# santurini/vsrlab

Hardware: AMD Instinct MI355X
Metric: LR frames/sec fwd+bwd, BasicVSR 4x 540p 7-frame clip, 1->8 MI355X (higher is better)
Workload: dtype bf16; 1 GPU; BasicVSR(mid=64,res_blocks=30,x4) fwd+Charbonnier+bwd+clip+Adam, 540x960->2160x3840, 7-frame clip, 2 clips per GPU (BASELINE configs[1]); clips_per_gpu=2, frames=7, res_blocks=30, parallelism=single GPU, arena=full, train_flow=False, trunk_chains=True

## Files before the change

### vsrlab_amd/csrc/conv3x3_c64_tile.h

```cpp
#pragma once
#include "common.h"

constexpr int PTW = 32, PTH = 8, PNT = 512;
constexpr int PTWH = PTW + 2, PTHH = PTH + 2, PNPIX = PTHH * PTWH;
constexpr int W_BYTES = 9 * 64 * 64 * 2;
constexpr int IN_BYTES = PNPIX * 128;
constexpr int BIAS_OFF = W_BYTES + 2 * IN_BYTES;
constexpr int IN_CHUNKS = PNPIX * 8;
constexpr int NPIECE_T = (IN_CHUNKS + 63) / 64;
constexpr int NPIECE_W = (NPIECE_T + 3) / 4;
constexpr int WCH = 9 * 64 * 8 / 256;

typedef __attribute__((ext_vector_type(2))) __bf16 bf16x2_t;
typedef __attribute__((ext_vector_type(4))) unsigned u32x4_t;
typedef __attribute__((ext_vector_type(2))) unsigned u32x2_t;
#define GP(T, x) ((__attribute__((address_space(1))) T*)(x))

static __device__ __forceinline__ unsigned pk_bf16(float a, float b) {
    bf16x2_t p = {(bf16_t)a, (bf16_t)b};
    return __builtin_bit_cast(unsigned, p);
}
static __device__ __forceinline__ unsigned pk_max_i16(unsigned a, unsigned b) { unsigned r; asm("v_pk_max_i16 %0, %1, %2" : "=v"(r) : "v"(a), "v"(b)); return r; }
static __device__ __forceinline__ unsigned pk_min_u16(unsigned a, unsigned b) { unsigned r; asm("v_pk_min_u16 %0, %1, %2" : "=v"(r) : "v"(a), "v"(b)); return r; }
static __device__ __forceinline__ unsigned pk_mul_lo_u16(unsigned a, unsigned b) { unsigned r; asm("v_pk_mul_lo_u16 %0, %1, %2" : "=v"(r) : "v"(a), "v"(b)); return r; }
// ... 12 lines not shown
        *reinterpret_cast<u32x4_t*>((lds_w) + tap * 8192 + C64_W_SWIZZLED_BYTE(r, c)) = wv[i];                           \
    }

#define C64_DMA_REL(rel, w4, lane, in_step, src_oy, src_ox, WSs)                                                         \
    _Pragma("unroll") for (int i = 0; i < NPIECE_W; ++i) {                                                               \
        const int idx = ((w4) + 4 * i) * 64 + (lane);             \
        const int ty = idx / (8 * PTWH), rem = idx - ty * (8 * PTWH);                                                    \
        const int c = rem / PTWH, tx = rem - c * PTWH;                                                                   \
        const int dx = (tx - 1) * (in_step) + (src_ox);                                                                  \
        rel[i] = (((((ty - 1) * (in_step) + (src_oy)) * (WSs) + (dx >> 5)) * 8 + c) * 256 + (dx & 31) * 8) * 2;          \
    }
#define C64_GLDS16(src, dst, AUX)                                                                     \
    __builtin_amdgcn_global_load_lds((const __attribute__((address_space(1))) void*)(src),            \
                                     (__attribute__((address_space(3))) void*)(dst), 16, 0, AUX)
#define C64_DMA_TILE(AUX, rel, org, zsrc, dstb, w4, lane, ty0, tx0, H, W)                                                \
    if (ty0 >= 1 && ty0 + PTH < (H) && tx0 >= 1 && tx0 + PTW < (W)) {                   \
        _Pragma("unroll") for (int i = 0; i < NPIECE_W; ++i) {                                                           \
            const int piece = (w4) + 4 * i;                                                                              \
            if (piece < NPIECE_T && piece * 64 + (lane) < IN_CHUNKS) C64_GLDS16((org) + rel[i], (dstb) + piece * 1024, AUX); \
        }                                                                                                                \
    } else {                                                                     \
        _Pragma("unroll") for (int i = 0; i < NPIECE_W; ++i) {                                                           \
            const int piece = (w4) + 4 * i;                                                                              \
            const int idx = piece * 64 + (lane);                                                                         \
            const int ty = idx / (8 * PTWH), rem = idx - ty * (8 * PTWH);                                                \
            const int tx = rem % PTWH;                                                                                   \
            const int vy = ty0 + ty - 1, vx = tx0 + tx - 1;                                                              \
            const auto* s = (vy >= 0 && vy < (H) && vx >= 0 && vx < (W)) ? (org) + rel[i] : (zsrc);                      \
            if (piece < NPIECE_T && idx < IN_CHUNKS) C64_GLDS16(s, (dstb) + piece * 1024, AUX);                          \
        }                                                                                                                \
    }

#define C64_MFMA_LANE(w4, l15, q, pxl)                                                                                   \
    unsigned a_lo[2], a_hi[2];                                                                                           \
    _Pragma("unroll") for (int kk = 0; kk < 2; ++kk) {                                                                   \
        a_lo[kk] = (unsigned)C64_W_SWIZZLED_BYTE(l15, 4 * kk + (q));                                                     \
        a_hi[kk] = a_lo[kk] + 6 * 8192;                                                                                  \
    }                                                                                                                    \
    const int b_lane = (w4) * 2 * (PTWH * 128) + (q) * (PTWH * 16) + (pxl) * 16;
static __device__ __forceinline__ f32x4_t c64_bias_rows(const char* smem, int q, int mb) {
    return *reinterpret_cast<const f32x4_t*>(smem + BIAS_OFF + (mb * 16 + 4 * q) * 4);
}
#define C64_RES_IDENTITY(idA, l15, q)                                                                                    \
    bf16x8_t idA[2];                                                                                                     \
    _Pragma("unroll") for (int hb = 0; hb < 2; ++hb)                                                                     \
        _Pragma("unroll") for (int j = 0; j < 8; ++j) idA[hb][j] = (bf16_t)(((q) == ((l15) >> 2) && j == 4 * hb + ((l15) & 3)) ? 1.f : 0.f);
#define C64_ADD_RESIDUAL(acc, idA, rr)                                                                                 \
    _Pragma("unroll") for (int nb = 0; nb < 4; ++nb)                                                                   \
        _Pragma("unroll") for (int mb = 0; mb < 4; ++mb)                                                               \
            acc[mb][nb] = __builtin_amdgcn_mfma_f32_16x16x32_bf16(idA[mb & 1], __builtin_bit_cast(bf16x8_t, rr[mb >> 1][nb]), acc[mb][nb], 0, 0, 0);

#define C64_DSR(dst, addr, imm) asm volatile("ds_read_b128 %0, %1 offset:%2" : "=v"(dst) : "v"(addr), "i"(imm))
#define C64_LOADA(tap_, kk_, slot, mb)                                                                                 \
    C64_DSR(fa_[slot][mb], (tap_ < 6 ? a_lo[kk_] : a_hi[kk_]), (tap_ < 6 ? tap_ : tap_ - 6) * 8192 + (mb) * 2048);
#define C64_LOADB(ky_, kx_, kk_, slot, nb)                                                                             \
    C64_DSR(fb_[slot][nb], bb_, (((nb) >> 1) + ky_) * (PTWH * 128) + kk_ * (4 * PTWH * 16) + (((nb) & 1) * 16 + kx_) * 16);
#define C64_LOAD(s, slot)                                                                                              \
    {                                                                                                                  \
        constexpr int tap_ = (s) / 2, kk_ = (s) % 2, ky_ = tap_ / 3, kx_ = tap_ % 3;                                   \
        C64_LOADA(tap_, kk_, slot, 0) C64_LOADA(tap_, kk_, slot, 1) C64_LOADA(tap_, kk_, slot, 2) C64_LOADA(tap_, kk_, slot, 3) \
        C64_LOADB(ky_, kx_, kk_, slot, 0) C64_LOADB(ky_, kx_, kk_, slot, 1) C64_LOADB(ky_, kx_, kk_, slot, 2) C64_LOADB(ky_, kx_, kk_, slot, 3) \
    }
#define C64_MFMA(acc, bvec, s, mb, nb) acc[mb][nb] = __builtin_amdgcn_mfma_f32_16x16x32_bf16(fa_[(s) % 2][mb], fb_[(s) % 2][nb], (s) == 0 ? bvec[mb] : acc[mb][nb], 0, 0, 0);
#define C64_ML_A(acc, bvec, s, mb, nb, lmb)                                                                            \
    C64_MFMA(acc, bvec, s, mb, nb)                                                                                     \
    __builtin_amdgcn_sched_barrier(0);                       \
    if ((s) + 1 < 18) { constexpr int t1_ = ((s) + 1) / 2, k1_ = ((s) + 1) % 2; C64_LOADA(t1_, k1_, ((s) + 1) % 2, lmb) } \
    __builtin_amdgcn_sched_barrier(0);
#define C64_ML_B(acc, bvec, s, mb, nb, lnb)                                                                            \
    C64_MFMA(acc, bvec, s, mb, nb)                                                                                     \
    __builtin_amdgcn_sched_barrier(0);                                                                                 \
    if ((s) + 1 < 18) { constexpr int t1_ = ((s) + 1) / 2, k1_ = ((s) + 1) % 2; C64_LOADB(t1_ / 3, t1_ % 3, k1_, ((s) + 1) % 2, lnb) } \
    __builtin_amdgcn_sched_barrier(0);
#define C64_STEP(acc, bvec, s)                                                                                         \
    {                                                                                                                  \
        asm volatile("s_waitcnt lgkmcnt(0)" ::: "memory");                                 \
        __builtin_amdgcn_sched_barrier(0);                                                                             \
        C64_ML_A(acc, bvec, s, 0, 0, 0) C64_ML_A(acc, bvec, s, 0, 1, 1) C64_ML_A(acc, bvec, s, 0, 2, 2) C64_ML_A(acc, bvec, s, 0, 3, 3) \
        C64_ML_B(acc, bvec, s, 1, 0, 0) C64_ML_B(acc, bvec, s, 1, 1, 1) C64_ML_B(acc, bvec, s, 1, 2, 2) C64_ML_B(acc, bvec, s, 1, 3, 3) \
        C64_MFMA(acc, bvec, s, 2, 0) C64_MFMA(acc, bvec, s, 2, 1) C64_MFMA(acc, bvec, s, 2, 2) C64_MFMA(acc, bvec, s, 2, 3)  \
        C64_MFMA(acc, bvec, s, 3, 0) C64_MFMA(acc, bvec, s, 3, 1) C64_MFMA(acc, bvec, s, 3, 2) C64_MFMA(acc, bvec, s, 3, 3)  \
        __builtin_amdgcn_sched_barrier(0);                                                                             \
    }
#define C64_K_LOOP(acc, bvec, cur)                                                                                                    \
    {                                                                                                                  \
        bf16x8_t fa_[2][4], fb_[2][4];                                                                                 \
        const unsigned bb_ = (unsigned)(W_BYTES + (cur) * IN_BYTES + (b_lane));      \
        asm volatile("s_waitcnt lgkmcnt(0)" ::: "memory");                         \
        __builtin_amdgcn_sched_barrier(0);                                                                             \
        C64_LOAD(0, 0)                                                                                                 \
        C64_STEP(acc, bvec, 0) C64_STEP(acc, bvec, 1) C64_STEP(acc, bvec, 2) C64_STEP(acc, bvec, 3) C64_STEP(acc, bvec, 4) C64_STEP(acc, bvec, 5) \
        C64_STEP(acc, bvec, 6) C64_STEP(acc, bvec, 7) C64_STEP(acc, bvec, 8) C64_STEP(acc, bvec, 9) C64_STEP(acc, bvec, 10) C64_STEP(acc, bvec, 11) \
        C64_STEP(acc, bvec, 12) C64_STEP(acc, bvec, 13) C64_STEP(acc, bvec, 14) C64_STEP(acc, bvec, 15) C64_STEP(acc, bvec, 16) C64_STEP(acc, bvec, 17) \
    }

constexpr unsigned C64_K11 = 0x00010001u;
#define C64_ARM_PLAIN(ow, v)                                                                                             \
    _Pragma("unroll") for (int jj = 0; jj < 4; ++jj) ow[jj] = pk_bf16(v[2 * jj], v[2 * jj + 1]);
#define C64_ARM_RELU(ow, v, nb, sign_k)                                                                                  \
    _Pragma("unroll") for (int jj = 0; jj < 4; ++jj) {                                                                   \
        ow[jj] = pk_max_i16(pk_bf16(v[2 * jj], v[2 * jj + 1]), 0u);                                                      \
        sign_k |= pk_min_u16(ow[jj], C64_K11) << (4 * (nb) + jj);                                                        \
    }
#define C64_ARM_MASKED(ow, v, nb, wbits)                                                                                 \
    _Pragma("unroll") for (int jj = 0; jj < 4; ++jj)                                                                     \
        ow[jj] = pk_mul_lo_u16(pk_bf16(v[2 * jj], v[2 * jj + 1]), ((wbits) >> (4 * (nb) + jj)) & C64_K11);
static __device__ __forceinline__ long long c64_sign_word(int tile, int w4, int lane) { return (long long)tile * 256 + w4 * 64 + lane; }
```

### vsrlab_amd/csrc/conv3x3_chain.hip

```cpp
#include "conv3x3_c64_tile.h"
#include "kernels.h"
#include <atomic>
#include <type_traits>

namespace {

constexpr int CTL_OFF = BIAS_OFF + 256;
constexpr int P_LDS = CTL_OFF + 128;
constexpr int DMA_SC1 = 16;

#ifdef VSR_CLOCK
__device__ unsigned long long g_clk_chain[256 * 2];
#endif
#ifdef VSR_TEST_CHAIN_NO_PUBLISH
#define CHAIN_PUBLISH 0
#else
#define CHAIN_PUBLISH 1
#endif
__device__ uint4 g_chain_zero_chunk[2];
__device__ unsigned g_chain_timeouts;

typedef __attribute__((address_space(1))) unsigned gu32;
#define RLX_AGENT __ATOMIC_RELAXED, __HIP_MEMORY_SCOPE_AGENT

// ... 150 lines not shown
                if (__builtin_amdgcn_readfirstlane(s1[5]) == 0) {
                    (void)halo_wait(flg0 + 4 * ((long long)(l1 - 1) * tiles + (long long)n1 * per), ty1, tx1, nty, ntx, lane, err);
                    if (leader && lane == 0) s1[5] = 1;
                }
                __builtin_amdgcn_fence(__ATOMIC_ACQUIRE, "wavefront");
                issue(l1, n1, ty1, tx1, (k + 1) & 1);
            }
            if (leader) {
                int* s2 = ctl + 8 * ((k + 2) % 3);
                int it2 = -1, l2 = 0, n2 = 0, ty2 = 0, tx2 = 0;
                bool ok2 = false;
                if (fetch) {
                    asm volatile("s_waitcnt vmcnt(11)" : "+v"(nx) :: "memory");
                    static_assert(NPIECE_W == 11, "the counted wait above");
                    if (__builtin_amdgcn_readfirstlane((int)nx) == -1) asm volatile("s_waitcnt vmcnt(0)" : "+v"(nx) :: "memory");
                    it2 = chain_item((unsigned)__builtin_amdgcn_readfirstlane((int)nx), own, R, tiles, ntx, ka.nlayers);
                    if (it2 >= 0) {
                        l2 = it2 / tiles; const int r = it2 - l2 * tiles; n2 = r / per; const int r2 = r - n2 * per; ty2 = r2 / ntx; tx2 = r2 - ty2 * ntx;
                        ok2 = l2 == 0 || halo_ready(flg0 + 4 * ((long long)(l2 - 1) * tiles + (long long)n2 * per), ty2, tx2, nty, ntx, lane);
                    }
                }
                if (lane == 0) { s2[0] = it2; s2[1] = l2; s2[2] = n2; s2[3] = ty2; s2[4] = tx2; s2[5] = ok2 ? 1 : 0; }
            }
            asm volatile("s_waitcnt vmcnt(0)" ::: "memory");
            __syncthreads();
        }
    } else {
        u32x4_t wv[WCH];
        {
            const auto* wg = GP(const u32x4_t, base + (unsigned long long)ka.layer[ctl[1]].w * 256ull);
            C64_W_LOAD(wv, wg, tid & 255)
        }
        C64_MFMA_LANE(w4, l15, q, pxl)
        unsigned loff[4];
#pragma unroll
        for (int nb = 0; nb < 4; ++nb) {
            const int dx = (nb & 1) * 16 + pxl;
            loff[nb] = (((((w4 * 2 + (nb >> 1))) * WS + (dx >> 5)) * 8 + q) * 256 + (dx & 31) * 8) * 2;
        }
        C64_W_STORE(wv, lds_w, tid & 255)
        if (tid < 64) {
            const unsigned bo = ka.layer[ctl[1]].bias;
            reinterpret_cast<float*>(smem + BIAS_OFF)[tid] = bo != 0xffffffffu ? GP(const float, base + (unsigned long long)bo * 256ull)[pm_acc_chan(tid >> 4, tid & 15)] : 0.f;
        }
        asm volatile("s_waitcnt vmcnt(0)" ::: "memory");
        __syncthreads();
        f32x4_t bvec[4];
#pragma unroll
        for (int mb = 0; mb < 4; ++mb) bvec[mb] = c64_bias_rows(smem, q, mb);
        C64_RES_IDENTITY(idA, l15, q)

        int cur_layer = __builtin_amdgcn_readfirstlane(ctl[1]);
        unsigned long long p_dst, p_res, p_sbits, p_sout;
        int variant;
        auto layer_ptrs = [&](int l) {
            const ChainLayer L = ka.layer[l];
            p_dst = (unsigned long long)base + (unsigned long long)L.dst * 256ull;
            p_res = (unsigned long long)base + (unsigned long long)L.res * 256ull;
            p_sbits = (unsigned long long)base + (unsigned long long)L.sbits * 256ull;
            p_sout = L.sout != 0xffffffffu ? (unsigned long long)base + (unsigned long long)L.sout * 256ull : 0ull;
            variant = L.variant;
        };
        layer_ptrs(cur_layer);

        bool pending = false;
        gu32* pend_cnt = nullptr;
        int cur = 0;
        int item = __builtin_amdgcn_readfirstlane(ctl[0]), layer = cur_layer, tn = __builtin_amdgcn_readfirstlane(ctl[2]);
        int tyi = __builtin_amdgcn_readfirstlane(ctl[3]), txi = __builtin_amdgcn_readfirstlane(ctl[4]);
        for (int k = 0; item >= 0; ++k) {
            const int* sn = ctl + 8 * ((k + 1) % 3);
            int nx_item = -1, nx_layer = 0, nx_n = 0, nx_ty = 0, nx_tx = 0, nx_ok = 0;
            if (layer != cur_layer) {
                cur_layer = layer;
                layer_ptrs(layer);
                __syncthreads();
#pragma unroll
                for (int mb = 0; mb < 4; ++mb) bvec[mb] = c64_bias_rows(smem, q, mb);
            }
            const int tile = item - layer * tiles;
            const int ty0 = tyi * PTH, tx0 = txi * PTW;
            const long long tbase = (long long)tn * img + pm_off(ty0, tx0, 0, W, 64);
            const bool full = ty0 + PTH <= H && tx0 + PTW <= W;
            bool ok[4];
#pragma unroll
            for (int nb = 0; nb < 4; ++nb) ok[nb] = (tx0 + (nb & 1) * 16 + pxl < W) && (ty0 + w4 * 2 + (nb >> 1) < H);
            gu32* const my_cnt = flg0 + 4 * (long long)item + w4;

            auto body = [&](auto VC) {
                constexpr int V = decltype(VC)::value;
                constexpr bool HAS_RES = V == CHAIN_SKIP, BITS = V == CHAIN_MASK;
                u32x4_t rr[2][4];
                u32x2_t sbits = {0u, 0u};
                if (BITS) sbits = GP(const u32x2_t, p_sbits)[c64_sign_word(tile, w4, lane)];
                if (HAS_RES) {
                    const unsigned long long rbase = p_res + (unsigned long long)tbase * 2ull;
#pragma unroll
                    for (int nb = 0; nb < 4; ++nb) {
                        const unsigned lo = loff[nb];
                        if (full) {
                            if (nb == 0) asm volatile("s_nop 4\n\tglobal_load_dwordx4 %0, %1, %2 sc1" : "=v"(rr[0][nb]) : "v"(lo), "s"(rbase) : "memory");
                            else asm volatile("global_load_dwordx4 %0, %1, %2 sc1" : "=v"(rr[0][nb]) : "v"(lo), "s"(rbase) : "memory");
                            asm volatile("global_load_dwordx4 %0, %1, %2 offset:2048 sc1" : "=v"(rr[1][nb]) : "v"(lo), "s"(rbase) : "memory");
                        } else {
                            rr[0][nb] = u32x4_t{0u, 0u, 0u, 0u}; rr[1][nb] = u32x4_t{0u, 0u, 0u, 0u};
                            if (ok[nb]) {
                                asm volatile("s_nop 4\n\tglobal_load_dwordx4 %0, %1, %2 sc1" : "+v"(rr[0][nb]) : "v"(lo), "s"(rbase) : "memory");
                                asm volatile("global_load_dwordx4 %0, %1, %2 offset:2048 sc1" : "+v"(rr[1][nb]) : "v"(lo), "s"(rbase) : "memory");
                            }
                        }
                    }
                }
                f32x4_t acc[4][4];
                C64_K_LOOP(acc, bvec, cur)
                nx_item = sn[0]; nx_layer = sn[1]; nx_n = sn[2]; nx_ty = sn[3]; nx_tx = sn[4]; nx_ok = sn[5];
                __builtin_amdgcn_s_waitcnt(0x0F70);
                __builtin_amdgcn_sched_barrier(0);
                if (pending) {
                    if (lane == 0 && CHAIN_PUBLISH) __hip_atomic_store(pend_cnt, 1u, RLX_AGENT);
                    pending = false;
                }
                if constexpr (HAS_RES) { C64_ADD_RESIDUAL(acc, idA, rr) }
                unsigned sout[2] = {0u, 0u};
                const unsigned long long dbase = p_dst + (unsigned long long)tbase * 2ull;
                auto epilogue = [&](auto FULL) {
                    const unsigned long long db = dbase;
#pragma unroll
                    for (int nb = 0; nb < 4; ++nb) {
                        if (decltype(FULL)::value || ok[nb]) {
                            const unsigned lo = loff[nb];
#pragma unroll
                            for (int kq = 0; kq < 2; ++kq) {
                                float v[8];
#pragma unroll
                                for (int j = 0; j < 4; ++j) { v[j] = acc[2 * kq][nb][j]; v[4 + j] = acc[2 * kq + 1][nb][j]; }
                                const unsigned wbits = kq ? sbits.y : sbits.x;
                                unsigned ow[4];
                                if (V == CHAIN_RELU) { C64_ARM_RELU(ow, v, nb, sout[kq]) }
                                else if (V == CHAIN_MASK) { C64_ARM_MASKED(ow, v, nb, wbits) }
                                else { C64_ARM_PLAIN(ow, v) }
                                const u32x4_t o = {ow[0], ow[1], ow[2], ow[3]};
                                if (kq == 0) {
                                    if (nb == 0 || !decltype(FULL)::value) asm volatile("s_nop 4\n\tglobal_store_dwordx4 %0, %1, %2 sc1\n\ts_nop 1" :: "v"(lo), "v"(o), "s"(db) : "memory");
                                    else asm volatile("global_store_dwordx4 %0, %1, %2 sc1\n\ts_nop 1" :: "v"(lo), "v"(o), "s"(db) : "memory");
                                } else asm volatile("global_store_dwordx4 %0, %1, %2 offset:2048 sc1\n\ts_nop 1" :: "v"(lo), "v"(o), "s"(db) : "memory");
                            }
                        }
                    }
                };
                if (full) epilogue(std::true_type{}); else epilogue(std::false_type{});
                if (V == CHAIN_RELU && p_sout) GP(u32x2_t, p_sout)[c64_sign_word(tile, w4, lane)] = u32x2_t{sout[0], sout[1]};
            };
            if (variant == CHAIN_SKIP) body(std::integral_constant<int, CHAIN_SKIP>{});
            else body(std::integral_constant<int, EVEN>{});

            pending = true; pend_cnt = my_cnt;
            if (nx_item < 0 || nx_ok == 0) {
                asm volatile("s_waitcnt vmcnt(0)" ::: "memory");
                if (lane == 0 && CHAIN_PUBLISH) __hip_atomic_store(pend_cnt, 1u, RLX_AGENT);
                pending = false;
            }
            __syncthreads();
            cur ^= 1;
            item = __builtin_amdgcn_readfirstlane(nx_item); layer = __builtin_amdgcn_readfirstlane(nx_layer); tn = __builtin_amdgcn_readfirstlane(nx_n);
            tyi = __builtin_amdgcn_readfirstlane(nx_ty); txi = __builtin_amdgcn_readfirstlane(nx_tx);
        }
    }
#ifdef VSR_CLOCK
    if (tid == 0 && blockIdx.x < 256) {
        g_clk_chain[blockIdx.x * 2 + 0] = __builtin_amdgcn_s_memtime() - clk_t0;
        g_clk_chain[blockIdx.x * 2 + 1] = __builtin_amdgcn_s_memrealtime() - clk_r0;
    }
#endif
}

__global__ void chain_poison_kernel(const unsigned* err, unsigned short* last_image) {
    if (__hip_atomic_load(err, RLX_AGENT) == 0u) return;
    for (int i = threadIdx.x; i < 32 * 64; i += blockDim.x) last_image[i] = 0x7fc0u;
}

}

#ifdef VSR_CLOCK
extern "C" int vsr_debug_read_clk_chain(unsigned long long* host_out) {
// ... 86 lines not shown
```

### vsrlab_amd/csrc/conv3x3_persist.hip

```cpp
#include "conv3x3_c64_tile.h"
#include <type_traits>

namespace {

constexpr int P_LDS = BIAS_OFF + 256;

__device__ uint4 g_conv_zero_chunk[2];

template <int ACT> __device__ __forceinline__ float p_act(float v, float slope) {
    if (ACT == ACT_RELU) return v > 0.f ? v : 0.f;
    if (ACT == ACT_LEAKY) return v > 0.f ? v : slope * v;
    return v;
}

#ifdef VSR_CLOCK
__device__ unsigned long long g_clk[256 * 4];
#endif

__device__ __forceinline__ void tile_coords(int tile, int ntx, int nty, int& n, int& ty0, int& tx0) {
    const int per = ntx * nty;
    n = tile / per;
    const int r = tile - n * per;
    const int ty = r / ntx;
    ty0 = ty * PTH;
// ... 56 lines not shown

    if (tid < 64) reinterpret_cast<float*>(smem + BIAS_OFF)[tid] = a.bias ? GP(const float, a.bias)[(long long)z * a.bias_zstride + pm_acc_chan(tid >> 4, tid & 15)] : 0.f;

    const auto* wg = GP(const u32x4_t, a.wpack + (unsigned long long)((long long)z * a.w_zstride) * 2);

    if (role == 1) {
        const auto* src = GP(const char, a.src0);
        const auto* zsrc = GP(const char, g_conv_zero_chunk);
        int rel[NPIECE_W];
        C64_DMA_REL(rel, w4, lane, a.in_step, a.src_oy0, a.src_ox0, WSs)
        auto issue = [&](const TileIter& it, int buf) {
            const int n = it.n, ty0 = it.ty * PTH, tx0 = it.tx * PTW;
            const auto* org = src + ((long long)n * a.src_nstride0 + pm_off(ty0 * a.in_step, tx0 * a.in_step, 0, a.Ws, 64)) * 2;
            char* dstb = lds_t + buf * IN_BYTES;
            C64_DMA_TILE(DMA_PLAIN, rel, org, zsrc, dstb, w4, lane, ty0, tx0, a.H, a.W)
        };
        int cur = 0;
        TileIter it;
        it.init(walk.first, walk.stride, ntx, nty);
        if (it.tile < walk.end) issue(it, 0);
        asm volatile("s_waitcnt vmcnt(0)" ::: "memory");
        __syncthreads();
        while (it.tile < walk.end) {
            it.advance(walk.stride, ntx, nty);
            if (it.tile < walk.end) issue(it, cur ^ 1);
            asm volatile("s_waitcnt vmcnt(0)" ::: "memory");
            __syncthreads();
            cur ^= 1;
        }
    } else {
        u32x4_t wv[WCH];
        C64_W_LOAD(wv, wg, tid)
        C64_MFMA_LANE(w4, l15, q, pxl)
        int loff[4];
#pragma unroll
        for (int nb = 0; nb < 4; ++nb) {
            const int dx = ((nb & 1) * 16 + pxl) * a.out_step + a.out_oxz;
            loff[nb] = ((((w4 * 2 + (nb >> 1)) * a.out_step) * WSd + (dx >> 5)) * 8 + q) * 256 + (dx & 31) * 8;
            if (a.unshuffle) {
                const int row = w4 * 2 + (nb >> 1), px = (nb & 1) * 16 + pxl;
                loff[nb] = (int)(((row & 1) * 2 + (px & 1)) * a.plane) + (((row >> 1) * pm_ws(a.Wd >> 1)) * 8 + q) * 256 + (px >> 1) * 8;
            }
        }
        C64_W_STORE(wv, lds_w, tid)
        asm volatile("s_waitcnt vmcnt(0)" ::: "memory");
        __syncthreads();
        auto* const dst_z = GP(bf16_t, a.dstz);
        const auto* const res_z = GP(const bf16_t, a.resz);
        const auto* const aux_z = GP(const bf16_t, a.auxz);
        const auto* const sbits_z = GP(const u32x2_t, a.sign_bitsz);
        auto* const sout_z = GP(u32x2_t, a.sign_outz);
        const float slope = vsr_slope(a.leaky_slope);

        f32x4_t bvec[4];
#pragma unroll
        for (int mb = 0; mb < 4; ++mb) bvec[mb] = c64_bias_rows(smem, q, mb);
        C64_RES_IDENTITY(idA, l15, q)
        static_assert(!HAS_RES || ACT == ACT_NONE, "the residual goes in on the matrix cores, ahead of any activation");

        int cur = 0;
        TileIter it;
        for (it.init(walk.first, walk.stride, ntx, nty); it.tile < walk.end; it.advance(walk.stride, ntx, nty)) {
            const int tile = it.tile, n = it.n, ty0 = it.ty * PTH, tx0 = it.tx * PTW;
            const long long tbase = a.unshuffle ? (long long)n * a.dst_nstride + pm_off(ty0 >> 1, tx0 >> 1, 0, a.Wd >> 1, 64)
                                                : (long long)n * a.dst_nstride + pm_off(ty0 * a.out_step + a.out_oyz, tx0 * a.out_step, 0, a.Wd, 64);
            const bool full = ty0 + PTH <= a.H && tx0 + PTW <= a.W;
            bool ok[4];
            constexpr bool BITS = MASK == MASK_RELU_BITS || MASK == MASK_LEAKY_BITS;
            constexpr bool LATE_MASK = HAS_RES && MASK != MASK_NONE && !BITS;
            u32x4_t rr[2][4], mm[2][4];
            u32x2_t sbits = {0u, 0u};
            if (BITS) sbits = sbits_z[c64_sign_word(tile, w4, lane)];
#pragma unroll
            for (int nb = 0; nb < 4; ++nb) ok[nb] = (tx0 + (nb & 1) * 16 + pxl < a.W) && (ty0 + w4 * 2 + (nb >> 1) < a.H);
#define CV_OPERANDS(OKN)                                                                                               \
            _Pragma("unroll") for (int nb = 0; nb < 4; ++nb) {                                                         \
                if (OKN) {                                                                                             \
                    _Pragma("unroll") for (int k = 0; k < 2; ++k) {                                                    \
                        const long long o = tbase + loff[nb] + k * 1024;                                               \
                        if (HAS_RES) rr[k][nb] = *GP(const u32x4_t, res_z + o);                                        \
                        if (MASK != MASK_NONE && !LATE_MASK && !BITS) mm[k][nb] = *GP(const u32x4_t, aux_z + o);       \
                    }                                                                                                  \
                }                                                                                                      \
            }
            if (HAS_RES || (MASK != MASK_NONE && !LATE_MASK && !BITS)) {
                if (full) { CV_OPERANDS(true) } else { CV_OPERANDS(ok[nb]) }
            }
#undef CV_OPERANDS

            f32x4_t acc[4][4];

            C64_K_LOOP(acc, bvec, cur)

            if (HAS_RES || MASK != MASK_NONE) __builtin_amdgcn_s_waitcnt(0x0F70);
            if constexpr (HAS_RES) { C64_ADD_RESIDUAL(acc, idA, rr) }
            unsigned sout[2] = {0u, 0u};
            auto epilogue = [&](auto FULL) {
#pragma unroll
            for (int nb = 0; nb < 4; ++nb) {
                if (decltype(FULL)::value || ok[nb]) {
                    auto* dst = dst_z + tbase + loff[nb];
#pragma unroll
                    for (int k = 0; k < 2; ++k) {
                        float v[8];
#pragma unroll
                        for (int j = 0; j < 4; ++j) { v[j] = acc[2 * k][nb][j]; v[4 + j] = acc[2 * k + 1][nb][j]; }
                        const unsigned wbits = k ? sbits.y : sbits.x;
                        unsigned ow[4];
                        if (ACT == ACT_RELU && !HAS_RES && MASK == MASK_NONE) {
                            C64_ARM_RELU(ow, v, nb, sout[k])
                        } else if (ACT == ACT_LEAKY && !HAS_RES && MASK == MASK_NONE) {
#pragma unroll
                            for (int jj = 0; jj < 4; ++jj) {
                                ow[jj] = pk_bf16(fmaxf(v[2 * jj], v[2 * jj] * slope), fmaxf(v[2 * jj + 1], v[2 * jj + 1] * slope));
                                sout[k] |= pk_min_u16(pk_max_i16(ow[jj], 0u), C64_K11) << (4 * nb + jj);
                            }
                        } else if (ACT == ACT_NONE && !HAS_RES && MASK == MASK_RELU_BITS) {
                            C64_ARM_MASKED(ow, v, nb, wbits)
                        } else {
#pragma unroll
                            for (int j = 0; j < 8; ++j) v[j] = p_act<ACT>(v[j], slope);
                            if (ACT != ACT_NONE && !HAS_RES) {
#pragma unroll
                                for (int j = 0; j < 8; ++j) sout[k] |= (v[j] > 0.f ? 1u : 0u) << (4 * nb + (j >> 1) + 16 * (j & 1));
                            }
                            if (BITS) {
                                const float neg = MASK == MASK_LEAKY_BITS ? slope : 0.f;
#pragma unroll
                                for (int j = 0; j < 8; ++j) v[j] *= ((wbits >> (4 * nb + (j >> 1) + 16 * (j & 1))) & 1u) ? 1.f : neg;
                            } else if (MASK != MASK_NONE) {
                                const float neg = MASK == MASK_LEAKY ? slope : 0.f;
                                u32x4_t mq = mm[k][nb];
                                if (LATE_MASK) mq = *GP(const u32x4_t, aux_z + tbase + loff[nb] + k * 1024);
                                const unsigned mw[4] = {mq.x, mq.y, mq.z, mq.w};
#pragma unroll
                                for (int jj = 0; jj < 4; ++jj) {
                                    v[2 * jj] *= (bf_lo(mw[jj]) > 0.f ? 1.f : neg);
                                    v[2 * jj + 1] *= (bf_hi(mw[jj]) > 0.f ? 1.f : neg);
                                }
                            }
                            C64_ARM_PLAIN(ow, v)
                        }
                        const u32x4_t o = {ow[0], ow[1], ow[2], ow[3]};
                        *GP(u32x4_t, dst + k * 1024) = o;
                    }
                }
            }
            };
            if (full) epilogue(std::true_type{}); else epilogue(std::false_type{});
            if (ACT != ACT_NONE && !HAS_RES && sout_z) sout_z[c64_sign_word(tile, w4, lane)] = u32x2_t{sout[0], sout[1]};
            __syncthreads();
            cur ^= 1;
        }
    }
#ifdef VSR_CLOCK
    if (tid == 0 && blockIdx.y == 0 && blockIdx.x < 256) {
        g_clk[blockIdx.x * 4 + 0] = __builtin_amdgcn_s_memtime() - clk_t0;
        g_clk[blockIdx.x * 4 + 1] = __builtin_amdgcn_s_memrealtime() - clk_r0;
    }
#endif
}

__global__ void sign_bits_c64_kernel(const bf16_t* __restrict__ x, uint2* __restrict__ bits, int N, int H, int W) {
    const int ntx = cdiv(W, PTW), nty = cdiv(H, PTH);
    const long long total = (long long)N * ntx * nty * 256;
    const long long gid = (long long)blockIdx.x * blockDim.x + threadIdx.x;
    if (gid >= total) return;
    const int lane = (int)(gid & 63), w4 = (int)((gid >> 6) & 3);
    const int tile = (int)(gid >> 8);
    const int l15 = lane & 15, q = lane >> 4;
    const int pxl = PM_LANE_PIXEL(l15);
    int n, ty0, tx0;
    tile_coords(tile, ntx, nty, n, ty0, tx0);
    unsigned out[2] = {0u, 0u};
#pragma unroll
    for (int nb = 0; nb < 4; ++nb) {
        const int yy = ty0 + 2 * w4 + (nb >> 1), xx = tx0 + (nb & 1) * 16 + pxl;
        if (yy < H && xx < W) {
#pragma unroll
            for (int k = 0; k < 2; ++k) {
                const uint4 v = *reinterpret_cast<const uint4*>(x + (long long)n * pm_image_elems(H, W, 64) + pm_off(yy, xx, 4 * k + q, W, 64));
                const unsigned vw[4] = {v.x, v.y, v.z, v.w};
#pragma unroll
// ... 77 lines not shown
```

Before: 59.87 LR frames/s.

## Split conv3x3 C64 wave tiles by output-channel half and four rows, reusing B across ky

Each of the four waves now owns half the output channels (2 M-blocks) over four pixel rows (8 N-blocks) instead of all 64 channels over two rows. This lets each loaded input row fragment be reused across the three vertical kernel taps. The K-loop is rewritten as a software pipeline with four rotating register slots and finer lgkmcnt waits, so LDS reads of the next step interleave with MFMAs. The goal is fewer LDS reads per MFMA and less stalling. In exchange the epilogue, residual, mask and sign-bit indexing become more complex, and the explicit waitcnt counts must be exactly right.

```diff
diff --git a/vsrlab_amd/csrc/conv3x3_c64_tile.h b/vsrlab_amd/csrc/conv3x3_c64_tile.h
--- a/vsrlab_amd/csrc/conv3x3_c64_tile.h
+++ b/vsrlab_amd/csrc/conv3x3_c64_tile.h
@@ -68,12 +68,13 @@
     }
 
 #define C64_MFMA_LANE(w4, l15, q, pxl)                                                                                   \
+    const int kh = (w4) & 1, rh = (w4) >> 1;                                                                             \
     unsigned a_lo[2], a_hi[2];                                                                                           \
     _Pragma("unroll") for (int kk = 0; kk < 2; ++kk) {                                                                   \
-        a_lo[kk] = (unsigned)C64_W_SWIZZLED_BYTE(l15, 4 * kk + (q));                                                     \
+        a_lo[kk] = (unsigned)(C64_W_SWIZZLED_BYTE(l15, 4 * kk + (q)) + kh * 4096);                                       \
         a_hi[kk] = a_lo[kk] + 6 * 8192;                                                                                  \
     }                                                                                                                    \
-    const int b_lane = (w4) * 2 * (PTWH * 128) + (q) * (PTWH * 16) + (pxl) * 16;
+    const int b_lane = rh * 4 * (PTWH * 128) + (q) * (PTWH * 16) + (pxl) * 16;
 static __device__ __forceinline__ f32x4_t c64_bias_rows(const char* smem, int q, int mb) {
     return *reinterpret_cast<const f32x4_t*>(smem + BIAS_OFF + (mb * 16 + 4 * q) * 4);
 }
@@ -82,52 +83,63 @@
     _Pragma("unroll") for (int hb = 0; hb < 2; ++hb)                                                                     \
         _Pragma("unroll") for (int j = 0; j < 8; ++j) idA[hb][j] = (bf16_t)(((q) == ((l15) >> 2) && j == 4 * hb + ((l15) & 3)) ? 1.f : 0.f);
 #define C64_ADD_RESIDUAL(acc, idA, rr)                                                                                 \
-    _Pragma("unroll") for (int nb = 0; nb < 4; ++nb)                                                                   \
-        _Pragma("unroll") for (int mb = 0; mb < 4; ++mb)                                                               \
-            acc[mb][nb] = __builtin_amdgcn_mfma_f32_16x16x32_bf16(idA[mb & 1], __builtin_bit_cast(bf16x8_t, rr[mb >> 1][nb]), acc[mb][nb], 0, 0, 0);
+    _Pragma("unroll") for (int nb = 0; nb < 8; ++nb)                                                                   \
+        _Pragma("unroll") for (int mb = 0; mb < 2; ++mb)                                                               \
+            acc[mb][nb] = __builtin_amdgcn_mfma_f32_16x16x32_bf16(idA[mb], __builtin_bit_cast(bf16x8_t, rr[nb]), acc[mb][nb], 0, 0, 0);
 
 #define C64_DSR(dst, addr, imm) asm volatile("ds_read_b128 %0, %1 offset:%2" : "=v"(dst) : "v"(addr), "i"(imm))
-#define C64_LOADA(tap_, kk_, slot, mb)                                                                                 \
-    C64_DSR(fa_[slot][mb], (tap_ < 6 ? a_lo[kk_] : a_hi[kk_]), (tap_ < 6 ? tap_ : tap_ - 6) * 8192 + (mb) * 2048);
-#define C64_LOADB(ky_, kx_, kk_, slot, nb)                                                                             \
-    C64_DSR(fb_[slot][nb], bb_, (((nb) >> 1) + ky_) * (PTWH * 128) + kk_ * (4 * PTWH * 16) + (((nb) & 1) * 16 + kx_) * 16);
-#define C64_LOAD(s, slot)                                                                                              \
+#define C64_RA(s, ky_, mb)                                                                                             \
+    if ((s) < 6) {                                                                                                     \
+        constexpr int tap_ = (ky_) * 3 + (s) / 2;                                                                      \
+        C64_DSR(fa_[(3 * (s) + (ky_)) & 3][mb], (tap_ < 6 ? a_lo[(s) % 2] : a_hi[(s) % 2]), (tap_ < 6 ? tap_ : tap_ - 6) * 8192 + (mb) * 2048); \
+    }
+#define C64_RB(s, j_, hf)                                                                                              \
+    if ((s) < 6) { C64_DSR(fb_[(6 * (s) + (j_)) & 3][hf], bb_, (j_) * (PTWH * 128) + ((s) % 2) * (4 * PTWH * 16) + ((hf) * 16 + (s) / 2) * 16); }
+#define C64_MM(acc, bvec, s, j_, ky_, mb, hf)                                                                          \
+    acc[mb][2 * ((j_) - (ky_)) + (hf)] = __builtin_amdgcn_mfma_f32_16x16x32_bf16(fa_[(3 * (s) + (ky_)) & 3][mb], fb_[(6 * (s) + (j_)) & 3][hf], \
+        ((s) == 0 && (ky_) == 0) ? bvec[mb] : acc[mb][2 * ((j_) - (ky_)) + (hf)], 0, 0, 0);
+#define C64_SB __builtin_amdgcn_sched_barrier(0);
+#define C64_PAIR(acc, bvec, s, j_, ky_)                                                                                \
+    C64_MM(acc, bvec, s, j_, ky_, 0, 0) C64_MM(acc, bvec, s, j_, ky_, 0, 1) C64_MM(acc, bvec, s, j_, ky_, 1, 0) C64_MM(acc, bvec, s, j_, ky_, 1, 1)
+#define C64_PAIR_R2(acc, bvec, s, j_, ky_, R0, R1)                                                                     \
+    C64_MM(acc, bvec, s, j_, ky_, 0, 0) C64_SB R0 C64_SB C64_MM(acc, bvec, s, j_, ky_, 0, 1) C64_SB R1 C64_SB          \
+    C64_MM(acc, bvec, s, j_, ky_, 1, 0) C64_MM(acc, bvec, s, j_, ky_, 1, 1)
+#define C64_PAIR_R4(acc, bvec, s, j_, ky_, R0, R1, R2, R3)                                                             \
+    C64_MM(acc, bvec, s, j_, ky_, 0, 0) C64_SB R0 C64_SB C64_MM(acc, bvec, s, j_, ky_, 0, 1) C64_SB R1 C64_SB          \
+    C64_MM(acc, bvec, s, j_, ky_, 1, 0) C64_SB R2 C64_SB C64_MM(acc, bvec, s, j_, ky_, 1, 1) C64_SB R3 C64_SB
+#define C64_WAIT(n, s, j_)                                                                                             \
+    if ((j_) < 3) asm volatile("s_waitcnt lgkmcnt(" #n ")" : "+v"(fb_[(6 * (s) + (j_)) & 3][0]), "+v"(fb_[(6 * (s) + (j_)) & 3][1]),     \
+                               "+v"(fa_[(3 * (s) + ((j_) % 3)) & 3][0]), "+v"(fa_[(3 * (s) + ((j_) % 3)) & 3][1]) :: "memory");           \
+    else asm volatile("s_waitcnt lgkmcnt(" #n ")" : "+v"(fb_[(6 * (s) + (j_)) & 3][0]), "+v"(fb_[(6 * (s) + (j_)) & 3][1]) :: "memory"); \
+    C64_SB
+#define C64_GROUPS(acc, bvec, s, W3, W4, W5)                                                                           \
     {                                                                                                                  \
-        constexpr int tap_ = (s) / 2, kk_ = (s) % 2, ky_ = tap_ / 3, kx_ = tap_ % 3;                                   \
-        C64_LOADA(tap_, kk_, slot, 0) C64_LOADA(tap_, kk_, slot, 1) C64_LOADA(tap_, kk_, slot, 2) C64_LOADA(tap_, kk_, slot, 3) \
-        C64_LOADB(ky_, kx_, kk_, slot, 0) C64_LOADB(ky_, kx_, kk_, slot, 1) C64_LOADB(ky_, kx_, kk_, slot, 2) C64_LOADB(ky_, kx_, kk_, slot, 3) \
+        C64_WAIT(8, s, 0)                                                                                              \
+        C64_PAIR_R2(acc, bvec, s, 0, 0, C64_RB(s, 3, 0), C64_RB(s, 3, 1))                                              \
+        C64_WAIT(6, s, 1)                                                                                              \
+        C64_PAIR_R2(acc, bvec, s, 1, 0, C64_RB(s, 4, 0), C64_RB(s, 4, 1)) C64_PAIR(acc, bvec, s, 1, 1)                  \
+        C64_WAIT(4, s, 2)                                                                                              \
+        C64_PAIR_R4(acc, bvec, s, 2, 0, C64_RB(s, 5, 0), C64_RB(s, 5, 1), C64_RA((s) + 1, 0, 0), C64_RA((s) + 1, 0, 1)) \
+        C64_PAIR(acc, bvec, s, 2, 1) C64_PAIR(acc, bvec, s, 2, 2)                                                      \
+        C64_WAIT(W3, s, 3)                                                                                             \
+        C64_PAIR_R2(acc, bvec, s, 3, 0, C64_RB((s) + 1, 0, 0), C64_RB((s) + 1, 0, 1)) C64_PAIR(acc, bvec, s, 3, 1) C64_PAIR(acc, bvec, s, 3, 2) \
+        C64_WAIT(W4, s, 4)                                                                                             \
+        C64_PAIR_R4(acc, bvec, s, 4, 1, C64_RB((s) + 1, 1, 0), C64_RB((s) + 1, 1, 1), C64_RA((s) + 1, 1, 0), C64_RA((s) + 1, 1, 1)) \
+        C64_PAIR(acc, bvec, s, 4, 2)                                                                                   \
+        C64_WAIT(W5, s, 5)                                                                                             \
+        C64_PAIR_R4(acc, bvec, s, 5, 2, C64_RB((s) + 1, 2, 0), C64_RB((s) + 1, 2, 1), C64_RA((s) + 1, 2, 0), C64_RA((s) + 1, 2, 1)) \
     }
-#define C64_MFMA(acc, bvec, s, mb, nb) acc[mb][nb] = __builtin_amdgcn_mfma_f32_16x16x32_bf16(fa_[(s) % 2][mb], fb_[(s) % 2][nb], (s) == 0 ? bvec[mb] : acc[mb][nb], 0, 0, 0);
-#define C64_ML_A(acc, bvec, s, mb, nb, lmb)                                                                            \
-    C64_MFMA(acc, bvec, s, mb, nb)                                                                                     \
-    __builtin_amdgcn_sched_barrier(0);                       \
-    if ((s) + 1 < 18) { constexpr int t1_ = ((s) + 1) / 2, k1_ = ((s) + 1) % 2; C64_LOADA(t1_, k1_, ((s) + 1) % 2, lmb) } \
-    __builtin_amdgcn_sched_barrier(0);
-#define C64_ML_B(acc, bvec, s, mb, nb, lnb)                                                                            \
-    C64_MFMA(acc, bvec, s, mb, nb)                                                                                     \
-    __builtin_amdgcn_sched_barrier(0);                                                                                 \
-    if ((s) + 1 < 18) { constexpr int t1_ = ((s) + 1) / 2, k1_ = ((s) + 1) % 2; C64_LOADB(t1_ / 3, t1_ % 3, k1_, ((s) + 1) % 2, lnb) } \
-    __builtin_amdgcn_sched_barrier(0);
-#define C64_STEP(acc, bvec, s)                                                                                         \
+#define C64_K_LOOP(acc, bvec, cur)                                                                                     \
     {                                                                                                                  \
-        asm volatile("s_waitcnt lgkmcnt(0)" ::: "memory");                                 \
-        __builtin_amdgcn_sched_barrier(0);                                                                             \
-        C64_ML_A(acc, bvec, s, 0, 0, 0) C64_ML_A(acc, bvec, s, 0, 1, 1) C64_ML_A(acc, bvec, s, 0, 2, 2) C64_ML_A(acc, bvec, s, 0, 3, 3) \
-        C64_ML_B(acc, bvec, s, 1, 0, 0) C64_ML_B(acc, bvec, s, 1, 1, 1) C64_ML_B(acc, bvec, s, 1, 2, 2) C64_ML_B(acc, bvec, s, 1, 3, 3) \
-        C64_MFMA(acc, bvec, s, 2, 0) C64_MFMA(acc, bvec, s, 2, 1) C64_MFMA(acc, bvec, s, 2, 2) C64_MFMA(acc, bvec, s, 2, 3)  \
-        C64_MFMA(acc, bvec, s, 3, 0) C64_MFMA(acc, bvec, s, 3, 1) C64_MFMA(acc, bvec, s, 3, 2) C64_MFMA(acc, bvec, s, 3, 3)  \
-        __builtin_amdgcn_sched_barrier(0);                                                                             \
-    }
-#define C64_K_LOOP(acc, bvec, cur)                                                                                                    \
-    {                                                                                                                  \
-        bf16x8_t fa_[2][4], fb_[2][4];                                                                                 \
+        bf16x8_t fa_[4][2], fb_[4][2];                                                                                 \
         const unsigned bb_ = (unsigned)(W_BYTES + (cur) * IN_BYTES + (b_lane));      \
-        asm volatile("s_waitcnt lgkmcnt(0)" ::: "memory");                         \
-        __builtin_amdgcn_sched_barrier(0);                                                                             \
-        C64_LOAD(0, 0)                                                                                                 \
-        C64_STEP(acc, bvec, 0) C64_STEP(acc, bvec, 1) C64_STEP(acc, bvec, 2) C64_STEP(acc, bvec, 3) C64_STEP(acc, bvec, 4) C64_STEP(acc, bvec, 5) \
-        C64_STEP(acc, bvec, 6) C64_STEP(acc, bvec, 7) C64_STEP(acc, bvec, 8) C64_STEP(acc, bvec, 9) C64_STEP(acc, bvec, 10) C64_STEP(acc, bvec, 11) \
-        C64_STEP(acc, bvec, 12) C64_STEP(acc, bvec, 13) C64_STEP(acc, bvec, 14) C64_STEP(acc, bvec, 15) C64_STEP(acc, bvec, 16) C64_STEP(acc, bvec, 17) \
+        __builtin_amdgcn_s_waitcnt(0xC07F);          \
+        C64_SB                                       \
+        C64_RA(0, 0, 0) C64_RA(0, 0, 1) C64_RB(0, 0, 0) C64_RB(0, 0, 1) C64_RA(0, 1, 0) C64_RA(0, 1, 1) C64_RB(0, 1, 0) C64_RB(0, 1, 1) \
+        C64_RA(0, 2, 0) C64_RA(0, 2, 1) C64_RB(0, 2, 0) C64_RB(0, 2, 1)                                                 \
+        C64_SB                                                                                                         \
+        C64_GROUPS(acc, bvec, 0, 6, 6, 8) C64_GROUPS(acc, bvec, 1, 6, 6, 8) C64_GROUPS(acc, bvec, 2, 6, 6, 8)          \
+        C64_GROUPS(acc, bvec, 3, 6, 6, 8) C64_GROUPS(acc, bvec, 4, 6, 6, 8) C64_GROUPS(acc, bvec, 5, 4, 2, 0)          \
     }
 
 constexpr unsigned C64_K11 = 0x00010001u;
diff --git a/vsrlab_amd/csrc/conv3x3_chain.hip b/vsrlab_amd/csrc/conv3x3_chain.hip
--- a/vsrlab_amd/csrc/conv3x3_chain.hip
+++ b/vsrlab_amd/csrc/conv3x3_chain.hip
@@ -206,11 +206,11 @@
             C64_W_LOAD(wv, wg, tid & 255)
         }
         C64_MFMA_LANE(w4, l15, q, pxl)
-        unsigned loff[4];
-#pragma unroll
-        for (int nb = 0; nb < 4; ++nb) {
+        unsigned loff[8];
+#pragma unroll
+        for (int nb = 0; nb < 8; ++nb) {
             const int dx = (nb & 1) * 16 + pxl;
-            loff[nb] = (((((w4 * 2 + (nb >> 1))) * WS + (dx >> 5)) * 8 + q) * 256 + (dx & 31) * 8) * 2;
+            loff[nb] = (((((rh * 4 + (nb >> 1))) * WS + (dx >> 5)) * 8 + q) * 256 + (dx & 31) * 8 + kh * 1024) * 2;
         }
         C64_W_STORE(wv, lds_w, tid & 255)
         if (tid < 64) {
@@ -219,9 +219,9 @@
         }
         asm volatile("s_waitcnt vmcnt(0)" ::: "memory");
         __syncthreads();
-        f32x4_t bvec[4];
-#pragma unroll
-        for (int mb = 0; mb < 4; ++mb) bvec[mb] = c64_bias_rows(smem, q, mb);
+        f32x4_t bvec[2];
+#pragma unroll
+        for (int mb = 0; mb < 2; ++mb) bvec[mb] = c64_bias_rows(smem, q, 2 * kh + mb);
         C64_RES_IDENTITY(idA, l15, q)
 
         int cur_layer = __builtin_amdgcn_readfirstlane(ctl[1]);
@@ -250,42 +250,41 @@
                 layer_ptrs(layer);
                 __syncthreads();
 #pragma unroll
-                for (int mb = 0; mb < 4; ++mb) bvec[mb] = c64_bias_rows(smem, q, mb);
+                for (int mb = 0; mb < 2; ++mb) bvec[mb] = c64_bias_rows(smem, q, 2 * kh + mb);
             }
             const int tile = item - layer * tiles;
             const int ty0 = tyi * PTH, tx0 = txi * PTW;
             const long long tbase = (long long)tn * img + pm_off(ty0, tx0, 0, W, 64);
             const bool full = ty0 + PTH <= H && tx0 + PTW <= W;
-            bool ok[4];
-#pragma unroll
-            for (int nb = 0; nb < 4; ++nb) ok[nb] = (tx0 + (nb & 1) * 16 + pxl < W) && (ty0 + w4 * 2 + (nb >> 1) < H);
+            bool ok[8];
+#pragma unroll
+            for (int nb = 0; nb < 8; ++nb) ok[nb] = (tx0 + (nb & 1) * 16 + pxl < W) && (ty0 + rh * 4 + (nb >> 1) < H);
             gu32* const my_cnt = flg0 + 4 * (long long)item + w4;
 
             auto body = [&](auto VC) {
                 constexpr int V = decltype(VC)::value;
                 constexpr bool HAS_RES = V == CHAIN_SKIP, BITS = V == CHAIN_MASK;
-                u32x4_t rr[2][4];
-                u32x2_t sbits = {0u, 0u};
-                if (BITS) sbits = GP(const u32x2_t, p_sbits)[c64_sign_word(tile, w4, lane)];
+                u32x4_t rr[8];
+                unsigned sbits[2] = {0u, 0u};
+                if (BITS) {
+#pragma unroll
+                    for (int i = 0; i < 2; ++i) sbits[i] = GP(const unsigned, p_sbits)[c64_sign_word(tile, 2 * rh + i, lane) * 2 + kh];
+                }
                 if (HAS_RES) {
                     const unsigned long long rbase = p_res + (unsigned long long)tbase * 2ull;
 #pragma unroll
-                    for (int nb = 0; nb < 4; ++nb) {
+                    for (int nb = 0; nb < 8; ++nb) {
                         const unsigned lo = loff[nb];
                         if (full) {
-                            if (nb == 0) asm volatile("s_nop 4\n\tglobal_load_dwordx4 %0, %1, %2 sc1" : "=v"(rr[0][nb]) : "v"(lo), "s"(rbase) : "memory");
-                            else asm volatile("global_load_dwordx4 %0, %1, %2 sc1" : "=v"(rr[0][nb]) : "v"(lo), "s"(rbase) : "memory");
-                            asm volatile("global_load_dwordx4 %0, %1, %2 offset:2048 sc1" : "=v"(rr[1][nb]) : "v"(lo), "s"(rbase) : "memory");
+                            if (nb == 0) asm volatile("s_nop 4\n\tglobal_load_dwordx4 %0, %1, %2 sc1" : "=v"(rr[nb]) : "v"(lo), "s"(rbase) : "memory");
+                            else asm volatile("global_load_dwordx4 %0, %1, %2 sc1" : "=v"(rr[nb]) : "v"(lo), "s"(rbase) : "memory");
                         } else {
-                            rr[0][nb] = u32x4_t{0u, 0u, 0u, 0u}; rr[1][nb] = u32x4_t{0u, 0u, 0u, 0u};
-                            if (ok[nb]) {
-                                asm volatile("s_nop 4\n\tglobal_load_dwordx4 %0, %1, %2 sc1" : "+v"(rr[0][nb]) : "v"(lo), "s"(rbase) : "memory");
-                                asm volatile("global_load_dwordx4 %0, %1, %2 offset:2048 sc1" : "+v"(rr[1][nb]) : "v"(lo), "s"(rbase) : "memory");
-                            }
+                            rr[nb] = u32x4_t{0u, 0u, 0u, 0u};
+                            if (ok[nb]) asm volatile("s_nop 4\n\tglobal_load_dwordx4 %0, %1, %2 sc1" : "+v"(rr[nb]) : "v"(lo), "s"(rbase) : "memory");
                         }
                     }
                 }
-                f32x4_t acc[4][4];
+                f32x4_t acc[2][8];
                 C64_K_LOOP(acc, bvec, cur)
                 nx_item = sn[0]; nx_layer = sn[1]; nx_n = sn[2]; nx_ty = sn[3]; nx_tx = sn[4]; nx_ok = sn[5];
                 __builtin_amdgcn_s_waitcnt(0x0F70);
@@ -300,30 +299,28 @@
                 auto epilogue = [&](auto FULL) {
                     const unsigned long long db = dbase;
 #pragma unroll
-                    for (int nb = 0; nb < 4; ++nb) {
+                    for (int nb = 0; nb < 8; ++nb) {
                         if (decltype(FULL)::value || ok[nb]) {
                             const unsigned lo = loff[nb];
-#pragma unroll
-                            for (int kq = 0; kq < 2; ++kq) {
-                                float v[8];
-#pragma unroll
-                                for (int j = 0; j < 4; ++j) { v[j] = acc[2 * kq][nb][j]; v[4 + j] = acc[2 * kq + 1][nb][j]; }
-                                const unsigned wbits = kq ? sbits.y : sbits.x;
-                                unsigned ow[4];
-                                if (V == CHAIN_RELU) { C64_ARM_RELU(ow, v, nb, sout[kq]) }
-                                else if (V == CHAIN_MASK) { C64_ARM_MASKED(ow, v, nb, wbits) }
-                                else { C64_ARM_PLAIN(ow, v) }
-                                const u32x4_t o = {ow[0], ow[1], ow[2], ow[3]};
-                                if (kq == 0) {
-                                    if (nb == 0 || !decltype(FULL)::value) asm volatile("s_nop 4\n\tglobal_store_dwordx4 %0, %1, %2 sc1\n\ts_nop 1" :: "v"(lo), "v"(o), "s"(db) : "memory");
-                                    else asm volatile("global_store_dwordx4 %0, %1, %2 sc1\n\ts_nop 1" :: "v"(lo), "v"(o), "s"(db) : "memory");
-                                } else asm volatile("global_store_dwordx4 %0, %1, %2 offset:2048 sc1\n\ts_nop 1" :: "v"(lo), "v"(o), "s"(db) : "memory");
-                            }
+                            float v[8];
+#pragma unroll
+                            for (int j = 0; j < 4; ++j) { v[j] = acc[0][nb][j]; v[4 + j] = acc[1][nb][j]; }
+                            const unsigned wbits = sbits[nb >> 2];
+                            unsigned ow[4];
+                            if (V == CHAIN_RELU) { C64_ARM_RELU(ow, v, nb & 3, sout[nb >> 2]) }
+                            else if (V == CHAIN_MASK) { C64_ARM_MASKED(ow, v, nb & 3, wbits) }
+                            else { C64_ARM_PLAIN(ow, v) }
+                            const u32x4_t o = {ow[0], ow[1], ow[2], ow[3]};
+                            if (nb == 0 || !decltype(FULL)::value) asm volatile("s_nop 4\n\tglobal_store_dwordx4 %0, %1, %2 sc1\n\ts_nop 1" :: "v"(lo), "v"(o), "s"(db) : "memory");
+                            else asm volatile("global_store_dwordx4 %0, %1, %2 sc1\n\ts_nop 1" :: "v"(lo), "v"(o), "s"(db) : "memory");
                         }
                     }
                 };
                 if (full) epilogue(std::true_type{}); else epilogue(std::false_type{});
-                if (V == CHAIN_RELU && p_sout) GP(u32x2_t, p_sout)[c64_sign_word(tile, w4, lane)] = u32x2_t{sout[0], sout[1]};
+                if (V == CHAIN_RELU && p_sout) {
+#pragma unroll
+                    for (int i = 0; i < 2; ++i) GP(unsigned, p_sout)[c64_sign_word(tile, 2 * rh + i, lane) * 2 + kh] = sout[i];
+                }
             };
             if (variant == CHAIN_SKIP) body(std::integral_constant<int, CHAIN_SKIP>{});
             else body(std::integral_constant<int, EVEN>{});
diff --git a/vsrlab_amd/csrc/conv3x3_persist.hip b/vsrlab_amd/csrc/conv3x3_persist.hip
--- a/vsrlab_amd/csrc/conv3x3_persist.hip
+++ b/vsrlab_amd/csrc/conv3x3_persist.hip
@@ -112,29 +112,29 @@
         u32x4_t wv[WCH];
         C64_W_LOAD(wv, wg, tid)
         C64_MFMA_LANE(w4, l15, q, pxl)
-        int loff[4];
-#pragma unroll
-        for (int nb = 0; nb < 4; ++nb) {
+        unsigned loff[8];
+#pragma unroll
+        for (int nb = 0; nb < 8; ++nb) {
             const int dx = ((nb & 1) * 16 + pxl) * a.out_step + a.out_oxz;
-            loff[nb] = ((((w4 * 2 + (nb >> 1)) * a.out_step) * WSd + (dx >> 5)) * 8 + q) * 256 + (dx & 31) * 8;
+            loff[nb] = (unsigned)(((((rh * 4 + (nb >> 1)) * a.out_step) * WSd + (dx >> 5)) * 8 + q) * 256 + (dx & 31) * 8 + kh * 1024) * 2u;
             if (a.unshuffle) {
-                const int row = w4 * 2 + (nb >> 1), px = (nb & 1) * 16 + pxl;
-                loff[nb] = (int)(((row & 1) * 2 + (px & 1)) * a.plane) + (((row >> 1) * pm_ws(a.Wd >> 1)) * 8 + q) * 256 + (px >> 1) * 8;
+                const int row = rh * 4 + (nb >> 1), px = (nb & 1) * 16 + pxl;
+                loff[nb] = (unsigned)((int)(((row & 1) * 2 + (px & 1)) * a.plane) + (((row >> 1) * pm_ws(a.Wd >> 1)) * 8 + q) * 256 + (px >> 1) * 8 + kh * 1024) * 2u;
             }
         }
         C64_W_STORE(wv, lds_w, tid)
         asm volatile("s_waitcnt vmcnt(0)" ::: "memory");
         __syncthreads();
-        auto* const dst_z = GP(bf16_t, a.dstz);
-        const auto* const res_z = GP(const bf16_t, a.resz);
-        const auto* const aux_z = GP(const bf16_t, a.auxz);
-        const auto* const sbits_z = GP(const u32x2_t, a.sign_bitsz);
-        auto* const sout_z = GP(u32x2_t, a.sign_outz);
+        auto* const dst_z = GP(char, a.dstz);
+        const auto* const res_z = GP(const char, a.resz);
+        const auto* const aux_z = GP(const char, a.auxz);
+        const auto* const sbits_z = GP(const unsigned, a.sign_bitsz);
+        auto* const sout_z = GP(unsigned, a.sign_outz);
         const float slope = vsr_slope(a.leaky_slope);
 
-        f32x4_t bvec[4];
-#pragma unroll
-        for (int mb = 0; mb < 4; ++mb) bvec[mb] = c64_bias_rows(smem, q, mb);
+        f32x4_t bvec[2];
+#pragma unroll
+        for (int mb = 0; mb < 2; ++mb) bvec[mb] = c64_bias_rows(smem, q, 2 * kh + mb);
         C64_RES_IDENTITY(idA, l15, q)
         static_assert(!HAS_RES || ACT == ACT_NONE, "the residual goes in on the matrix cores, ahead of any activation");
 
@@ -145,22 +145,22 @@
             const long long tbase = a.unshuffle ? (long long)n * a.dst_nstride + pm_off(ty0 >> 1, tx0 >> 1, 0, a.Wd >> 1, 64)
                                                 : (long long)n * a.dst_nstride + pm_off(ty0 * a.out_step + a.out_oyz, tx0 * a.out_step, 0, a.Wd, 64);
             const bool full = ty0 + PTH <= a.H && tx0 + PTW <= a.W;
-            bool ok[4];
+            bool ok[8];
             constexpr bool BITS = MASK == MASK_RELU_BITS || MASK == MASK_LEAKY_BITS;
             constexpr bool LATE_MASK = HAS_RES && MASK != MASK_NONE && !BITS;
-            u32x4_t rr[2][4], mm[2][4];
-            u32x2_t sbits = {0u, 0u};
-            if (BITS) sbits = sbits_z[c64_sign_word(tile, w4, lane)];
-#pragma unroll
-            for (int nb = 0; nb < 4; ++nb) ok[nb] = (tx0 + (nb & 1) * 16 + pxl < a.W) && (ty0 + w4 * 2 + (nb >> 1) < a.H);
+            u32x4_t rr[8], mm[8];
+            unsigned sbits[2] = {0u, 0u};
+            if (BITS) {
+#pragma unroll
+                for (int i = 0; i < 2; ++i) sbits[i] = sbits_z[c64_sign_word(tile, 2 * rh + i, lane) * 2 + kh];
+            }
+#pragma unroll
+            for (int nb = 0; nb < 8; ++nb) ok[nb] = (tx0 + (nb & 1) * 16 + pxl < a.W) && (ty0 + rh * 4 + (nb >> 1) < a.H);
 #define CV_OPERANDS(OKN)                                                                                               \
-            _Pragma("unroll") for (int nb = 0; nb < 4; ++nb) {                                                         \
+            _Pragma("unroll") for (int nb = 0; nb < 8; ++nb) {                                                         \
                 if (OKN) {                                                                                             \
-                    _Pragma("unroll") for (int k = 0; k < 2; ++k) {                                                    \
-                        const long long o = tbase + loff[nb] + k * 1024;                                               \
-                        if (HAS_RES) rr[k][nb] = *GP(const u32x4_t, res_z + o);                                        \
-                        if (MASK != MASK_NONE && !LATE_MASK && !BITS) mm[k][nb] = *GP(const u32x4_t, aux_z + o);       \
-                    }                                                                                                  \
+                    if (HAS_RES) rr[nb] = *GP(const u32x4_t, res_z + tbase * 2 + loff[nb]);                            \
+                    if (MASK != MASK_NONE && !LATE_MASK && !BITS) mm[nb] = *GP(const u32x4_t, aux_z + tbase * 2 + loff[nb]); \
                 }                                                                                                      \
             }
             if (HAS_RES || (MASK != MASK_NONE && !LATE_MASK && !BITS)) {
@@ -168,7 +168,7 @@
             }
 #undef CV_OPERANDS
 
-            f32x4_t acc[4][4];
+            f32x4_t acc[2][8];
 
             C64_K_LOOP(acc, bvec, cur)
 
@@ -177,58 +177,59 @@
             unsigned sout[2] = {0u, 0u};
             auto epilogue = [&](auto FULL) {
 #pragma unroll
-            for (int nb = 0; nb < 4; ++nb) {
+            for (int nb = 0; nb < 8; ++nb) {
                 if (decltype(FULL)::value || ok[nb]) {
-                    auto* dst = dst_z + tbase + loff[nb];
-#pragma unroll
-                    for (int k = 0; k < 2; ++k) {
-                        float v[8];
-#pragma unroll
-                        for (int j = 0; j < 4; ++j) { v[j] = acc[2 * k][nb][j]; v[4 + j] = acc[2 * k + 1][nb][j]; }
-                        const unsigned wbits = k ? sbits.y : sbits.x;
-                        unsigned ow[4];
-                        if (ACT == ACT_RELU && !HAS_RES && MASK == MASK_NONE) {
-                            C64_ARM_RELU(ow, v, nb, sout[k])
-                        } else if (ACT == ACT_LEAKY && !HAS_RES && MASK == MASK_NONE) {
+                    auto* dst = dst_z + tbase * 2 + loff[nb];
+                    const int sb = 4 * (nb & 3);
+                    float v[8];
+#pragma unroll
+                    for (int j = 0; j < 4; ++j) { v[j] = acc[0][nb][j]; v[4 + j] = acc[1][nb][j]; }
+                    const unsigned wbits = sbits[nb >> 2];
+                    unsigned ow[4];
+                    if (ACT == ACT_RELU && !HAS_RES && MASK == MASK_NONE) {
+                        C64_ARM_RELU(ow, v, nb & 3, sout[nb >> 2])
+                    } else if (ACT == ACT_LEAKY && !HAS_RES && MASK == MASK_NONE) {
+#pragma unroll
+                        for (int jj = 0; jj < 4; ++jj) {
+                            ow[jj] = pk_bf16(fmaxf(v[2 * jj], v[2 * jj] * slope), fmaxf(v[2 * jj + 1], v[2 * jj + 1] * slope));
+                            sout[nb >> 2] |= pk_min_u16(pk_max_i16(ow[jj], 0u), C64_K11) << (sb + jj);
+                        }
+                    } else if (ACT == ACT_NONE && !HAS_RES && MASK == MASK_RELU_BITS) {
+                        C64_ARM_MASKED(ow, v, nb & 3, wbits)
+                    } else {
+#pragma unroll
+                        for (int j = 0; j < 8; ++j) v[j] = p_act<ACT>(v[j], slope);
+                        if (ACT != ACT_NONE && !HAS_RES) {
+#pragma unroll
+                            for (int j = 0; j < 8; ++j) sout[nb >> 2] |= (v[j] > 0.f ? 1u : 0u) << (sb + (j >> 1) + 16 * (j & 1));
+                        }
+                        if (BITS) {
+                            const float neg = MASK == MASK_LEAKY_BITS ? slope : 0.f;
+#pragma unroll
+                            for (int j = 0; j < 8; ++j) v[j] *= ((wbits >> (sb + (j >> 1) + 16 * (j & 1))) & 1u) ? 1.f : neg;
+                        } else if (MASK != MASK_NONE) {
+                            const float neg = MASK == MASK_LEAKY ? slope : 0.f;
+                            u32x4_t mq = mm[nb];
+                            if (LATE_MASK) mq = *GP(const u32x4_t, aux_z + tbase * 2 + loff[nb]);
+                            const unsigned mw[4] = {mq.x, mq.y, mq.z, mq.w};
 #pragma unroll
                             for (int jj = 0; jj < 4; ++jj) {
-                                ow[jj] = pk_bf16(fmaxf(v[2 * jj], v[2 * jj] * slope), fmaxf(v[2 * jj + 1], v[2 * jj + 1] * slope));
-                                sout[k] |= pk_min_u16(pk_max_i16(ow[jj], 0u), C64_K11) << (4 * nb + jj);
+                                v[2 * jj] *= (bf_lo(mw[jj]) > 0.f ? 1.f : neg);
+                                v[2 * jj + 1] *= (bf_hi(mw[jj]) > 0.f ? 1.f : neg);
                             }
-                        } else if (ACT == ACT_NONE && !HAS_RES && MASK == MASK_RELU_BITS) {
-                            C64_ARM_MASKED(ow, v, nb, wbits)
-                        } else {
-#pragma unroll
-                            for (int j = 0; j < 8; ++j) v[j] = p_act<ACT>(v[j], slope);
-                            if (ACT != ACT_NONE && !HAS_RES) {
-#pragma unroll
-                                for (int j = 0; j < 8; ++j) sout[k] |= (v[j] > 0.f ? 1u : 0u) << (4 * nb + (j >> 1) + 16 * (j & 1));
-                            }
-                            if (BITS) {
-                                const float neg = MASK == MASK_LEAKY_BITS ? slope : 0.f;
-#pragma unroll
-                                for (int j = 0; j < 8; ++j) v[j] *= ((wbits >> (4 * nb + (j >> 1) + 16 * (j & 1))) & 1u) ? 1.f : neg;
-                            } else if (MASK != MASK_NONE) {
-                                const float neg = MASK == MASK_LEAKY ? slope : 0.f;
-                                u32x4_t mq = mm[k][nb];
-                                if (LATE_MASK) mq = *GP(const u32x4_t, aux_z + tbase + loff[nb] + k * 1024);
-                                const unsigned mw[4] = {mq.x, mq.y, mq.z, mq.w};
-#pragma unroll
-                                for (int jj = 0; jj < 4; ++jj) {
-                                    v[2 * jj] *= (bf_lo(mw[jj]) > 0.f ? 1.f : neg);
-                                    v[2 * jj + 1] *= (bf_hi(mw[jj]) > 0.f ? 1.f : neg);
-                                }
-                            }
-                            C64_ARM_PLAIN(ow, v)
                         }
-                        const u32x4_t o = {ow[0], ow[1], ow[2], ow[3]};
-                        *GP(u32x4_t, dst + k * 1024) = o;
+                        C64_ARM_PLAIN(ow, v)
                     }
+                    const u32x4_t o = {ow[0], ow[1], ow[2], ow[3]};
+                    *GP(u32x4_t, dst) = o;
                 }
             }
             };
             if (full) epilogue(std::true_type{}); else epilogue(std::false_type{});
-            if (ACT != ACT_NONE && !HAS_RES && sout_z) sout_z[c64_sign_word(tile, w4, lane)] = u32x2_t{sout[0], sout[1]};
+            if (ACT != ACT_NONE && !HAS_RES && sout_z) {
+#pragma unroll
+                for (int i = 0; i < 2; ++i) sout_z[c64_sign_word(tile, 2 * rh + i, lane) * 2 + kh] = sout[i];
+            }
             __syncthreads();
             cur ^= 1;
         }
```

Result: no change. 60.32 LR frames/s (median of 6 runs) (+0.8%).
